# PARKCHEOLHEE-lab/building-gan-graph-conditioned-architectural-volume-generation

Measured on AMD Instinct MI355X. Metric: voxel-graphs/sec (full G+D step), higher is better.
Workload: dtype f32

## Files before the change

### building-gan-graph-conditioned-architectural-volume-generation_amd/csrc/gemm.hip

```cpp
#include "gemm_tile.h"

namespace {

using namespace vg::tile;

typedef float f32x16 __attribute__((ext_vector_type(16)));
typedef __bf16 bf16x4 __attribute__((ext_vector_type(4)));
typedef __bf16 bf16x8 __attribute__((ext_vector_type(8)));

constexpr int LDH = TK + 8;

__device__ __forceinline__ bf16x4 to_bf4(const float (&v)[4]) {
  bf16x4 r;
  r[0] = static_cast<__bf16>(v[0]);
  r[1] = static_cast<__bf16>(v[1]);
  r[2] = static_cast<__bf16>(v[2]);
  r[3] = static_cast<__bf16>(v[3]);
  return r;
}

__device__ __forceinline__ f32x16 mfma_bf(const __bf16* a, const __bf16* b, f32x16 acc) {
  return __builtin_amdgcn_mfma_f32_32x32x16_bf16(*reinterpret_cast<const bf16x8*>(a),
                                                 *reinterpret_cast<const bf16x8*>(b), acc, 0, 0, 0);
}
// ... 522 lines not shown
__global__ void __launch_bounds__(1024) k_gemm16(const float* __restrict__ A, int lda, const float* __restrict__ B,
                                                 int ldb, const float* __restrict__ bias,
                                                 const float* __restrict__ aux, int ldaux, float* __restrict__ C,
                                                 int ldc, int N, int M, int K,
                                                 const float* __restrict__ att_s = nullptr,
                                                 const float* __restrict__ att_d = nullptr,
                                                 float* __restrict__ a_src = nullptr,
                                                 float* __restrict__ a_dst = nullptr, const GnpDesc gn = GnpDesc{}) {
  gemm16_body<BT, ACT, ATT, BF, GNP, false, QA>(A, lda, B, ldb, bias, aux, ldaux, C, ldc, N, M, K, att_s, att_d,
                                                a_src, a_dst, gn);
}

template <bool BT, int ACT, bool ATT = false, bool BF = false, bool GNP = false, bool QA = false>
__global__ void __launch_bounds__(512) k_gemm8w(const float* __restrict__ A, int lda, const float* __restrict__ B,
                                                int ldb, const float* __restrict__ bias,
                                                const float* __restrict__ aux, int ldaux, float* __restrict__ C,
                                                int ldc, int N, int M, int K,
                                                const float* __restrict__ att_s = nullptr,
                                                const float* __restrict__ att_d = nullptr,
                                                float* __restrict__ a_src = nullptr,
                                                float* __restrict__ a_dst = nullptr, const GnpDesc gn = GnpDesc{}) {
  gemm16_body<BT, ACT, ATT, BF, GNP, false, QA, 8>(A, lda, B, ldb, bias, aux, ldaux, C, ldc, N, M, K, att_s, att_d,
                                                   a_src, a_dst, gn);
}

__global__ void __launch_bounds__(1024) __attribute__((amdgpu_waves_per_eu(8, 8)))
k_gemm16_gna(const float* __restrict__ A, const float* __restrict__ B, float* __restrict__ C, int N, int M, int K,
             const float* __restrict__ att_s, const float* __restrict__ att_d, float* __restrict__ a_src,
             float* __restrict__ a_dst, const GnaDesc ga) {
  gemm16_body<true, 0, true, false, false, true>(A, K, B, K, nullptr, nullptr, 0, C, M, N, M, K, att_s, att_d,
                                                 a_src, a_dst, GnpDesc{}, ga);
}

template <int NT, int TMR, bool ATT, int NTH>
__device__ __forceinline__ void ln_tile_epilogue(const float* Ct, float* s_mu, float* s_rs, int t, int n0, int N,
                                                 int M, const float* __restrict__ gamma,
                                                 const float* __restrict__ beta, float eps, float slope,
                                                 float* __restrict__ H, float* __restrict__ Y,
                                                 float* __restrict__ mean, float* __restrict__ rstd,
                                                 const float* __restrict__ att_s, const float* __restrict__ att_d,
                                                 float* __restrict__ a_src, float* __restrict__ a_dst, int ldy,
                                                 int s0 = 0) {
  constexpr int TNC = TN * NT;
  constexpr int CT = TNC + 1;
  if constexpr (ATT) {
    constexpr int TPR = NTH / TMR;
    constexpr int CPT = TNC / TPR;
    const int row = t / TPR, q = t % TPR;
    const float* cr = Ct + row * CT + q * CPT;
    float ss = 0.f, sd = 0.f;
#pragma unroll
    for (int i = 0; i < CPT; ++i) {
      const int c = q * CPT + i;
      if (c < M) {
        ss = fmaf(cr[i], att_s[c], ss);
        sd = fmaf(cr[i], att_d[c], sd);
      }
    }
#pragma unroll
    for (int off = 1; off < TPR; off <<= 1) {
      ss += __shfl_xor(ss, off, 64);
      sd += __shfl_xor(sd, off, 64);
    }
    if (q == 0 && n0 + row < N) {
      a_src[n0 + row] = ss;
      a_dst[n0 + row] = sd;
    }
    for (int idx = t; idx < TMR * TNC; idx += NTH) {
      const int r = idx / TNC, c = idx % TNC, n = n0 + r;
      if (c < M && n < N) H[(size_t)n * M + c] = Ct[r * CT + c];
    }
    return;
  }
  {
    constexpr int TPR = NTH / TMR;
    constexpr int CPT = TNC / TPR;
    const int row = t / TPR, q = t % TPR;
    const float* cr = Ct + row * CT + q * CPT;
    float v[CPT];
    float s = 0.f;
#pragma unroll
    for (int i = 0; i < CPT; ++i) {
      v[i] = q * CPT + i < M ? cr[i] : 0.f;
      s += v[i];
    }
#pragma unroll
    for (int off = 1; off < TPR; off <<= 1) s += __shfl_xor(s, off, 64);
    const float mu = s / static_cast<float>(M);
    float ss = 0.f;
#pragma unroll
    for (int i = 0; i < CPT; ++i)
      if (q * CPT + i < M) {
        const float d = v[i] - mu;
        ss = fmaf(d, d, ss);
      }
#pragma unroll
    for (int off = 1; off < TPR; off <<= 1) ss += __shfl_xor(ss, off, 64);
    const float rs = rsqrtf(ss / static_cast<float>(M) + eps);
    if (q == 0) {
      s_mu[row] = mu;
      s_rs[row] = rs;
      if (mean && n0 + row < N && n0 + row >= s0) {
        mean[n0 + row - s0] = mu;
        rstd[n0 + row - s0] = rs;
      }
    }
  }
  __syncthreads();
  for (int idx = t; idx < TMR * TNC; idx += NTH) {
    const int row = idx / TNC, c = idx % TNC, n = n0 + row;
    if (c < M && n < N) {
      const float v = Ct[row * CT + c];
      if (H && n >= s0) H[(size_t)(n - s0) * M + c] = v;
      const float z = fmaf((v - s_mu[row]) * s_rs[row], gamma[c], beta[c]);
      Y[(size_t)n * ldy + c] = z > 0.f ? z : z * slope;
    }
  }
}

constexpr int kMaxSrc = 4;
struct MsDesc {
  const float* p[kMaxSrc];
  int ld[kMaxSrc], kend[kMaxSrc], wcol[kMaxSrc], rmod[kMaxSrc];
  int nsrc;
  const float* add;
  int ld_add, add_rows;
  int s0 = 0;
};

template <int NT, int TMR = TM, bool ATT = false, bool MS = false, bool BF = false, bool QL = false>
__global__ void __launch_bounds__(256) k_gemm_ln(const float* __restrict__ A, int lda,
                                                 const float* __restrict__ B, int ldb,
                                                 const float* __restrict__ bias, int N, int M, int K,
                                                 const float* __restrict__ gamma,
                                                 const float* __restrict__ beta, float eps,
                                                 float slope, float* __restrict__ H,
                                                 float* __restrict__ Y, float* __restrict__ mean,
                                                 float* __restrict__ rstd,
                                                 const float* __restrict__ att_s = nullptr,
                                                 const float* __restrict__ att_d = nullptr,
                                                 float* __restrict__ a_src = nullptr,
                                                 float* __restrict__ a_dst = nullptr, int ldy = 0,
                                                 const MsDesc ms = MsDesc{}) {
  if (ldy == 0) ldy = M;
  constexpr int TNC = TN * NT;
  constexpr int CT = TNC + 1;
  constexpr int WCOLS = 4 / (TMR / 32);
  constexpr int NJ = TNC / (32 * WCOLS);
  static_assert(NJ >= 1, "TMR = 32 needs 128 columns");
  __shared__ __attribute__((aligned(16))) float smem[2 * TMR * LDP + 2 * TNC * LDP];
  __shared__ float s_mu[TMR], s_rs[TMR];
// ... 289 lines not shown
      const float* ar = As + buf * TMR * PIT + (wr * 16 + (lane & 15)) * LDP + (lane >> 4);
#pragma unroll
      for (int kk = 0; kk < TK; kk += 4)
#pragma unroll
        for (int j = 0; j < NJ; ++j)
          acc[j] = __builtin_amdgcn_mfma_f32_16x16x4f32(
              ar[kk], Bs[buf * TNC * PIT + (j * 16 * WCW + wc * 16 + (lane & 15)) * LDP + (lane >> 4) + kk], acc[j], 0,
              0, 0);
    }
    buf ^= 1;
  }
  __syncthreads();
  float* Ct = smem;
  const int add0 = MS && ms.add ? n0 % ms.add_rows : 0;
#pragma unroll
  for (int j = 0; j < NJ; ++j) {
    const int c = j * 16 * WCW + wc * 16 + (lane & 15);
    const float bv = (bias && c < M) ? bias[c] : 0.f;
#pragma unroll
    for (int r = 0; r < 4; ++r) {
      const int rl = wr * 16 + 4 * (lane >> 4) + r;
      float v = acc[j][r] + bv;
      if constexpr (MS) {
        if (ms.add && n0 + rl < N && c < M) {
          int ar2 = add0 + rl;
          if (ar2 >= ms.add_rows) ar2 -= ms.add_rows;
          v += ms.add[(size_t)ar2 * ms.ld_add + c];
        }
      }
      Ct[rl * CT + c] = v;
    }
  }
  __syncthreads();
  ln_tile_epilogue<NT, TMR, ATT, 1024>(Ct, s_mu, s_rs, t, n0, N, M, gamma, beta, eps, slope, H, Y, mean, rstd, att_s,
                                       att_d, a_src, a_dst, ldy, ms.s0);
}

template <int KT, bool MS>
__global__ void __launch_bounds__(1024) k_gemm_ln_wres(const float* __restrict__ A, int lda,
                                                       const float* __restrict__ B, int ldb,
                                                       const float* __restrict__ bias, int N, int M, int K,
                                                       const float* __restrict__ gamma,
                                                       const float* __restrict__ beta, float eps, float slope,
                                                       float* __restrict__ H, float* __restrict__ Y,
                                                       float* __restrict__ mean, float* __restrict__ rstd, int ldy,
                                                       const MsDesc ms) {
  constexpr int TMR = 32, NT = 2, TNC = TN * NT, CT = TNC + 1;
  constexpr int WRW = TMR / 16, WCW = 16 / WRW;
  static_assert(TNC / (16 * WCW) == 1, "one sub-tile per wave");
  constexpr int AIMG = TMR * FP, BIMG = TNC * FP;
  extern __shared__ float4 dyn4[];
  float* Ws = reinterpret_cast<float*>(dyn4);
  float* As = Ws + KT * BIMG;
  __shared__ float s_mu[TMR], s_rs[TMR];
  const int t = threadIdx.x, lane = t & 63, wave = t >> 6;
  const int wr = wave / WCW, wc = wave % WCW;
  const int kq4 = K / 4;
  const int tiles = (N + TMR - 1) / TMR;
  const int lb = xcd_remap(blockIdx.x, gridDim.x);
  const int t0 = (int)((long long)tiles * lb / gridDim.x), t1 = (int)((long long)tiles * (lb + 1) / gridDim.x);
  auto a_src = [&](int k, const float*& p, int& ld, int& col) {
    p = A;
    ld = lda;
    col = k;
    if constexpr (MS) {
      int sidx = 0;
#pragma unroll
      for (int i = 0; i < kMaxSrc - 1; ++i)
        if (i < ms.nsrc - 1 && k >= ms.kend[i]) sidx = i + 1;
      const int kb = sidx > 0 ? ms.kend[sidx - 1] : 0;
      p = ms.p[sidx];
      ld = ms.ld[sidx];
      col = k - kb;
    }
  };
  auto w_col = [&](int k) {
    if constexpr (MS) {
      int sidx = 0;
#pragma unroll
      for (int i = 0; i < kMaxSrc - 1; ++i)
        if (i < ms.nsrc - 1 && k >= ms.kend[i]) sidx = i + 1;
      const int kb = sidx > 0 ? ms.kend[sidx - 1] : 0;
      return ms.wcol[sidx] + (k - kb);
    }
    return k;
  };
  for (int g = t; g < TNC * kq4; g += 1024) {
    const int m = g / kq4, k = 4 * (g % kq4);
    const float4 v = m < M ? *reinterpret_cast<const float4*>(B + (size_t)m * ldb + w_col(k)) : make_float4(0.f, 0.f, 0.f, 0.f);
    float* d = Ws + (k >> 5) * BIMG;
    const int kk = k & 31;
    d[frag_pos(m, kk)] = v.x;
    d[frag_pos(m, kk + 1)] = v.y;
    d[frag_pos(m, kk + 2)] = v.z;
    d[frag_pos(m, kk + 3)] = v.w;
  }
  for (int g = t; g < TNC * (KT * 32 - K); g += 1024) {
    const int m = g / (KT * 32 - K), k = K + g % (KT * 32 - K);
    Ws[(k >> 5) * BIMG + frag_pos(m, k & 31)] = 0.f;
  }
  constexpr int QPT = (TMR * KT * 8 + 1023) / 1024;
  float4 qa[QPT];
  auto load_a = [&](int tile) {
    const int n0 = tile * TMR;
#pragma unroll
    for (int u = 0; u < QPT; ++u) {
      const int g = t + 1024 * u;
      const int r = g / kq4, k = 4 * (g % kq4);
      qa[u] = make_float4(0.f, 0.f, 0.f, 0.f);
      if (g < TMR * kq4 && n0 + r < N) {
        const float* p;
        int ld, col;
        a_src(k, p, ld, col);
        qa[u] = *reinterpret_cast<const float4*>(p + (size_t)(n0 + r) * ld + col);
      }
    }
  };
  auto store_a = [&]() {
#pragma unroll
    for (int u = 0; u < QPT; ++u) {
      const int g = t + 1024 * u;
      if (g < TMR * kq4) {
        const int r = g / kq4, k = 4 * (g % kq4);
        float* d = As + (k >> 5) * AIMG;
        const int kk = k & 31;
        d[frag_pos(r, kk)] = qa[u].x;
        d[frag_pos(r, kk + 1)] = qa[u].y;
        d[frag_pos(r, kk + 2)] = qa[u].z;
        d[frag_pos(r, kk + 3)] = qa[u].w;
      }
    }
    for (int g = t; g < TMR * (KT * 32 - K); g += 1024) {
      const int r = g / (KT * 32 - K), k = K + g % (KT * 32 - K);
      As[(k >> 5) * AIMG + frag_pos(r, k & 31)] = 0.f;
    }
  };
  if (t0 < t1) {
    load_a(t0);
    store_a();
  }
  const int c = wc * 16 + (lane & 15);
  const float bv = (bias && c < M) ? bias[c] : 0.f;
  __syncthreads();
  for (int tile = t0; tile < t1; ++tile) {
    const int n0 = tile * TMR;
    if (tile + 1 < t1) load_a(tile + 1);
    f32x4 acc = f32x4{0.f, 0.f, 0.f, 0.f};
    const int ra_ = wr * 16 + (lane & 15), g = lane >> 4;
#pragma unroll
    for (int kt = 0; kt < KT; ++kt) {
      const float* Ai = As + kt * AIMG;
      const float* Bi = Ws + kt * BIMG;
      const float4 a0 = *reinterpret_cast<const float4*>(Ai + frag_at(ra_, g, 0));
      const float4 a1 = *reinterpret_cast<const float4*>(Ai + frag_at(ra_, g, 1));
      const float av[8] = {a0.x, a0.y, a0.z, a0.w, a1.x, a1.y, a1.z, a1.w};
      const float4 b0 = *reinterpret_cast<const float4*>(Bi + frag_at(c, g, 0));
      const float4 b1 = *reinterpret_cast<const float4*>(Bi + frag_at(c, g, 1));
      const float bw[8] = {b0.x, b0.y, b0.z, b0.w, b1.x, b1.y, b1.z, b1.w};
#pragma unroll
      for (int i = 0; i < 8; ++i) acc = __builtin_amdgcn_mfma_f32_16x16x4f32(av[i], bw[i], acc, 0, 0, 0);
    }
    __syncthreads();
    float* Ct = As;
    const int add0 = MS && ms.add ? n0 % ms.add_rows : 0;
#pragma unroll
    for (int r = 0; r < 4; ++r) {
      const int rl = wr * 16 + 4 * (lane >> 4) + r;
      float v = acc[r] + bv;
      if constexpr (MS) {
        if (ms.add && n0 + rl < N && c < M) {
          int ar2 = add0 + rl;
          if (ar2 >= ms.add_rows) ar2 -= ms.add_rows;
          v += ms.add[(size_t)ar2 * ms.ld_add + c];
        }
      }
      Ct[rl * CT + c] = v;
    }
    __syncthreads();
    ln_tile_epilogue<NT, TMR, false, 1024>(Ct, s_mu, s_rs, t, n0, N, M, gamma, beta, eps, slope, H, Y, mean, rstd,
                                           nullptr, nullptr, nullptr, nullptr, ldy, ms.s0);
    __syncthreads();
    if (tile + 1 < t1) store_a();
    __syncthreads();
  }
}

template <int KT>
constexpr int wres_lds_bytes() {
  return (KT * TN * 2 * FP + (KT * 32 * FP > 32 * (2 * TN + 1) ? KT * 32 * FP : 32 * (2 * TN + 1))) * 4;
}

template <int G>
constexpr int tn_smem_floats() { return G * 2 * TK * (TM + 1) + G * 2 * TK * (TN + 1); }

template <int G, bool BF>
__device__ __forceinline__ void tn_tile(float* smem, const float* __restrict__ A, int lda, const float* __restrict__ B,
                                        int ldb, int N, int M, int K, int rows, int chunk, int m0, int k0,
                                        float* __restrict__ part, float* __restrict__ pdb, int db_rows) {
  float(*As)[2][TK][TM + 1] = reinterpret_cast<float(*)[2][TK][TM + 1]>(smem);
  float(*Bs)[2][TK][TN + 1] = reinterpret_cast<float(*)[2][TK][TN + 1]>(smem + G * 2 * TK * (TM + 1));
  constexpr int PER = (TK * TM) / 256;
  const int grp = threadIdx.x >> 8, t = threadIdx.x & 255, lane = t & 63, wave = t >> 6;
  const int wr = wave >> 1, wc = wave & 1;
  const int nb = chunk * rows, ne = min(N, nb + rows);
  const int steps = ne > nb ? (ne - nb + TK - 1) / TK : 0;
  const int iters = (steps + G - 1) / G;
  const bool do_db = pdb && k0 == 0;
  f32x16 acc;
#pragma unroll
  for (int r = 0; r < 16; ++r) acc[r] = 0.f;
  float dbs = 0.f;
  __bf16(*Ah)[2][TM][LDH] = reinterpret_cast<__bf16(*)[2][TM][LDH]>(smem);
  __bf16(*Bh)[2][TN][LDH] = reinterpret_cast<__bf16(*)[2][TN][LDH]>(smem + G * 2 * TK * (TM + 1));
  float ra[PER], rb[PER];
  auto load = [&](int st) {
    const int n1 = nb + st * TK;
#pragma unroll
    for (int q = 0; q < PER; ++q) {
      const int e = t + 256 * q;
      const int c = e % TM;
      const int r = BF ? 4 * ((t >> 6) + 4 * (q >> 2)) + (q & 3) : e / TM;
      const int n = n1 + r;
// ... 789 lines not shown
    k_gemm_tn_group<kTnGroups, true><<<static_cast<int>(blocks), 256 * kTnGroups, 0, s>>>(g);
  else
    k_gemm_tn_group<kTnGroups, false><<<static_cast<int>(blocks), 256 * kTnGroups, 0, s>>>(g);
  VG_CHECK_LAUNCH();
  return 0;
}

static inline bool al16(const void* p) { return (reinterpret_cast<uintptr_t>(p) & 15) == 0; }

#ifndef VG_WRES
#define VG_WRES 1
#endif
#ifndef VG_LN_TM64_K
#define VG_LN_TM64_K 384
#endif
#ifndef VG_WRES_MIN_ROWS
#define VG_WRES_MIN_ROWS 16384
#endif
static int wres_cus() {
  static int cus = 0;
  if (!cus) {
    int dev = 0, n = 0;
    if (hipGetDevice(&dev) != hipSuccess || hipDeviceGetAttribute(&n, hipDeviceAttributeMultiprocessorCount, dev) !=
                                                  hipSuccess || n <= 0)
      n = 256;
    cus = n;
  }
  return cus;
}

template <int KT, bool MS>
static void launch_wres(const float* A, int lda, const float* W, int ldw, const float* bias, int N, int M, int K,
                        const float* gamma, const float* beta, float eps, float slope, float* H, float* Y, float* mean,
                        float* rstd, int ldy, const MsDesc& d, hipStream_t s) {
  static bool attr = false;
  constexpr int bytes = wres_lds_bytes<KT>();
  if (!attr) {
    (void)hipFuncSetAttribute(reinterpret_cast<const void*>(&k_gemm_ln_wres<KT, MS>),
                              hipFuncAttributeMaxDynamicSharedMemorySize, bytes);
    attr = true;
  }
  const int tiles = (N + 31) / 32;
  const int grid = tiles < wres_cus() ? tiles : wres_cus();
  k_gemm_ln_wres<KT, MS><<<grid, 1024, bytes, s>>>(A, lda, W, ldw, bias, N, M, K, gamma, beta, eps, slope, H, Y, mean,
                                                   rstd, ldy, d);
}

template <bool MS>
static bool try_wres(const float* A, int lda, const float* W, int ldw, const float* bias, int N, int M, int K,
                     const float* gamma, const float* beta, float eps, float slope, float* H, float* Y, float* mean,
                     float* rstd, int ldy, const MsDesc& d, hipStream_t s) {
  if (!VG_WRES || N < VG_WRES_MIN_ROWS || M <= TN || M > 2 * TN || K % 4 || K <= 0) return false;
  switch ((K + 31) / 32) {
    case 1: launch_wres<1, MS>(A, lda, W, ldw, bias, N, M, K, gamma, beta, eps, slope, H, Y, mean, rstd, ldy, d, s); return true;
    case 2: launch_wres<2, MS>(A, lda, W, ldw, bias, N, M, K, gamma, beta, eps, slope, H, Y, mean, rstd, ldy, d, s); return true;
    case 3: launch_wres<3, MS>(A, lda, W, ldw, bias, N, M, K, gamma, beta, eps, slope, H, Y, mean, rstd, ldy, d, s); return true;
    case 4: launch_wres<4, MS>(A, lda, W, ldw, bias, N, M, K, gamma, beta, eps, slope, H, Y, mean, rstd, ldy, d, s); return true;
    case 5: launch_wres<5, MS>(A, lda, W, ldw, bias, N, M, K, gamma, beta, eps, slope, H, Y, mean, rstd, ldy, d, s); return true;
    default: return false;
  }
}

template <bool BF>
static int gemm_ln_act(const float* A, int32_t lda, const float* W, int32_t N, int32_t M,
                       int32_t K, const float* bias, const float* gamma, const float* beta,
                       float eps, float slope, float* H, float* Y, float* mean, float* rstd,
                       void* stream, int32_t s0 = 0) {
  if (N < 0 || M <= 0 || M > 2 * TN || K <= 0 || lda < K || !A || !W || !gamma || !beta || !Y ||
      ((mean == nullptr) != (rstd == nullptr)) || s0 < 0 || (s0 > 0 && s0 >= N))
    return VG_EINVAL;
  MsDesc d{};
  d.s0 = s0;
  if (N == 0) return 0;
  hipStream_t s = static_cast<hipStream_t>(stream);
  const dim3 grid((N + TM - 1) / TM, 1);
  const bool ql = VG_QUAD_A && K % 4 == 0 && lda % 4 == 0 && al16(A) && al16(W);
  if (!BF && ql && try_wres<false>(A, lda, W, K, bias, N, M, K, gamma, beta, eps, slope, H, Y, mean, rstd, M, d, s)) {
  } else if (!BF && VG_LN16) {
    if (M <= TN && ql)
      k_gemm_ln16<1, TM, false, false, true><<<grid, 1024, 0, s>>>(A, lda, W, K, bias, N, M, K, gamma, beta, eps,
                                                                  slope, H, Y, mean, rstd,
                                                                  nullptr, nullptr, nullptr, nullptr, 0, d);
    else if (M <= TN)
      k_gemm_ln16<1, TM><<<grid, 1024, 0, s>>>(A, lda, W, K, bias, N, M, K, gamma, beta, eps, slope, H, Y, mean,
                                              rstd, nullptr, nullptr, nullptr, nullptr, 0, d);
    else if (VG_LN_TM32 && ql && K >= VG_LN_TM64_K)
      k_gemm_ln16<2, TM, false, false, true><<<grid, 1024, 0, s>>>(A, lda, W, K, bias, N, M, K, gamma, beta, eps,
                                                                  slope, H, Y, mean, rstd,
                                                                  nullptr, nullptr, nullptr, nullptr, 0, d);
    else if (VG_LN_TM32 && ql)
      k_gemm_ln16<2, 32, false, false, true><<<dim3((N + 31) / 32, 1), 1024, 0, s>>>(
          A, lda, W, K, bias, N, M, K, gamma, beta, eps, slope, H, Y, mean, rstd,
          nullptr, nullptr, nullptr, nullptr, 0, d);
// ... 89 lines not shown
        nullptr, nullptr, ldy, d);
  else if (!BF && VG_LN16)
    k_gemm_ln16<2, 32, false, true><<<dim3((N + 31) / 32, 1), 1024, 0, s>>>(
        nullptr, 0, W, ldw, bias, N, M, K, gamma, beta, eps, slope, nullptr, Y, nullptr, nullptr, nullptr, nullptr,
        nullptr, nullptr, ldy, d);
  else if (BF && ql)
    k_gemm_ln<2, 32, false, true, BF, BF><<<dim3((N + 31) / 32, 1), 256, 0, s>>>(
        nullptr, 0, W, ldw, bias, N, M, K, gamma, beta, eps, slope, nullptr, Y, nullptr, nullptr, nullptr, nullptr,
        nullptr, nullptr, ldy, d);
  else
    k_gemm_ln<2, 32, false, true, BF><<<dim3((N + 31) / 32, 1), 256, 0, s>>>(
        nullptr, 0, W, ldw, bias, N, M, K, gamma, beta, eps, slope, nullptr, Y, nullptr, nullptr, nullptr, nullptr,
        nullptr, nullptr, ldy, d);
  VG_CHECK_LAUNCH();
  return 0;
}

extern "C" int vg_gemm_ln_act_ms(const vg_asrc* src, int32_t nsrc, const float* W, int32_t ldw, int32_t N,
                                 int32_t M, const float* bias, const float* addend, int32_t ld_add,
                                 int32_t add_rows, const float* gamma, const float* beta, float eps, float slope,
                                 float* Y, int32_t ldy, void* stream) {
  return gemm_ln_act_ms<false>(src, nsrc, W, ldw, N, M, bias, addend, ld_add, add_rows, gamma, beta, eps, slope,
                               Y, ldy, stream);
}

extern "C" int vg_gemm_ln_act_ms_bf16(const vg_asrc* src, int32_t nsrc, const float* W, int32_t ldw, int32_t N,
                                      int32_t M, const float* bias, const float* addend, int32_t ld_add,
                                      int32_t add_rows, const float* gamma, const float* beta, float eps,
                                      float slope, float* Y, int32_t ldy, void* stream) {
  return gemm_ln_act_ms<true>(src, nsrc, W, ldw, N, M, bias, addend, ld_add, add_rows, gamma, beta, eps, slope,
                              Y, ldy, stream);
}

template <bool BF>
static int gat_lin_att(const float* X, int32_t ldx, const float* W, int32_t N,
                       int32_t Cin, int32_t C, const float* att_src, const float* att_dst,
                       float* H, float* a_src, float* a_dst, void* stream) {
  if (N < 0 || Cin <= 0 || C <= 0 || ldx < Cin || !X || !W || !att_src || !att_dst || !H ||
      !a_src || !a_dst)
    return VG_EINVAL;
  if (N == 0) return 0;
  hipStream_t s = static_cast<hipStream_t>(stream);
  if (C > 2 * TN) {
    const int rc = gemm<BF>(X, ldx, W, Cin, 1, nullptr, 0, nullptr, 0, H, C, N, C, Cin, stream);
    if (rc) return rc;
    return vg_gat_att(H, N, C, att_src, att_dst, a_src, a_dst, stream);
  }
  if (C > TN) {
    if (!BF && VG_LN16 && quad_ab(X, ldx, W, Cin, Cin, C, true))
      k_gemm_ln16<2, 32, true, false, true><<<dim3((N + 31) / 32, 1), 1024, 0, s>>>(
          X, ldx, W, Cin, nullptr, N, C, Cin, nullptr, nullptr, 0.f, 0.f, H, nullptr, nullptr, nullptr, att_src,
          att_dst, a_src, a_dst);
    else if (!BF && VG_LN16)
      k_gemm_ln16<2, 32, true><<<dim3((N + 31) / 32, 1), 1024, 0, s>>>(
          X, ldx, W, Cin, nullptr, N, C, Cin, nullptr, nullptr, 0.f, 0.f, H, nullptr, nullptr, nullptr, att_src,
          att_dst, a_src, a_dst);
    else
      k_gemm_ln<2, 32, true, false, BF><<<dim3((N + 31) / 32, 1), 256, 0, s>>>(
          X, ldx, W, Cin, nullptr, N, C, Cin, nullptr, nullptr, 0.f, 0.f, H, nullptr, nullptr, nullptr, att_src,
          att_dst, a_src, a_dst);
    VG_CHECK_LAUNCH();
    return 0;
  }
  if ((VG_GEMM16 & 2) && (!BF || (VG_GEMM16 & 8)))
    if (quad_ab(X, ldx, W, Cin, Cin, C, true))
      if (use_8w(dim3((N + TM - 1) / TM, 1)))
// ... 93 lines not shown
```

### building-gan-graph-conditioned-architectural-volume-generation_amd/vgan/_lib.py

```python
from __future__ import annotations

import ctypes
import os
from typing import Optional

import torch

LIB_PATH = os.environ.get("VGAN_LIB") or os.path.join(os.path.dirname(os.path.abspath(__file__)), "libvgan_hip.so")
VG_EINVAL = -1
VG_SELECT_MAX_COPIES = 64
VG_SELECT_F1, VG_SELECT_FAR = 0, 1

_c_i32, _c_i64, _c_f32, _c_p = ctypes.c_int32, ctypes.c_int64, ctypes.c_float, ctypes.c_void_p



class VgFoldSrc(ctypes.Structure):
    _fields_ = [("part", _c_p), ("rows", _c_i32), ("ld", _c_i32)]


class VgFold(ctypes.Structure):
    _fields_ = [("out", _c_p), ("width", _c_i32), ("k", _c_i32), ("ldo", _c_i32), ("accumulate", _c_i32),
                ("nsrc", _c_i32), ("src", VgFoldSrc * 2)]

# ... 247 lines not shown
                                       _c_p, _c_p, _c_p]),
    "vg_hgat_gna_max_segments": (_c_i32, []),
    "vg_hgat_lin_att_gn": (ctypes.c_int, [_c_p, _c_i32, _c_p, _c_i32, _c_i32, _c_i32, _c_i32, _c_p, _c_p, _c_p,
                                          _c_i32, _c_p, _c_p, _c_p, _c_p, _c_p, _c_p, _c_i32, _c_i32, _c_i32, _c_p]),
    "vg_hgat_fwd": (ctypes.c_int, [_c_p, _c_p, _c_i32, _c_i32, _c_i32, _c_p, _c_p, _c_p, _c_p, _c_f32, _c_p, _c_i32,
                                   _c_p]),
    "vg_graphnorm_fwd_h": (ctypes.c_int, [_c_p, _c_i32, _c_i32, _c_i32, _c_i32, _c_p, _c_p, _c_p, _c_f32, _c_p,
                                          _c_i32, _c_p, _c_p, _c_p]),
    "vg_hgat_gnp_rows": (_c_i32, [_c_i32, _c_i32]),
    "vg_hgat_gnp_floats": (_c_i64, [_c_i32, _c_i32]),
    "vg_hgat_fwd_gnp": (ctypes.c_int, [_c_p, _c_p, _c_i32, _c_i32, _c_i32, _c_p, _c_p, _c_p, _c_p, _c_f32, _c_p,
                                       _c_i32, _c_i32, _c_p, _c_p]),
    "vg_graphnorm_fwd_h_gnp": (ctypes.c_int, [_c_p, _c_i32, _c_i32, _c_i32, _c_i32, _c_p, _c_p, _c_p, _c_f32, _c_p,
                                              _c_i32, _c_p, _c_p, _c_i32, _c_p]),
    "vg_rng_fill": (ctypes.c_int, [_c_p, _c_i64, _c_i32, ctypes.c_uint64, _c_p, ctypes.c_uint32, _c_p]),
    "vg_rng_fill_at": (ctypes.c_int, [_c_p, _c_i64, _c_i32, ctypes.c_uint64, _c_p, _c_i64, ctypes.c_uint32, _c_p]),
    "vg_graphnorm_fwd_drop_tail": (ctypes.c_int, [_c_p, _c_i32, _c_i32, _c_i32, _c_p, _c_p, _c_p, _c_f32,
                                                  ctypes.c_uint64, _c_p, ctypes.c_uint32, _c_f32, _c_p, _c_p, _c_p, _c_p,
                                                  ctypes.POINTER(VgDrawTail), _c_p]),
    "vg_graphnorm_fwd_gnp_tail": (ctypes.c_int, [_c_p, _c_i32, _c_i32, _c_i32, _c_p, _c_p, _c_p, _c_f32,
                                                 ctypes.c_uint64, _c_p, ctypes.c_uint32, _c_f32, _c_p, _c_p, _c_p, _c_p,
                                                 _c_i32, ctypes.POINTER(VgDrawTail), _c_p]),
    "vg_gemm_ln_act_from": (ctypes.c_int, [_c_p, _c_i32, _c_p, _c_i32, _c_i32, _c_i32, _c_p, _c_p, _c_p, _c_f32,
                                           _c_f32, _c_i32, _c_p, _c_p, _c_p, _c_p, _c_p]),
    "vg_gen_state_bytes": (ctypes.c_int64, []),
    "vg_gen_hoist_arena_floats": (ctypes.c_int64, [ctypes.POINTER(VgGenModel), ctypes.POINTER(VgGenBatch),
                                                   ctypes.POINTER(VgGenStack)]),
    "vg_gen_forward_stacked": (ctypes.c_int, [ctypes.POINTER(VgGenModel), ctypes.POINTER(VgGenBatch),
                                              ctypes.POINTER(VgGenStack), _c_p, _c_i64, _c_p, _c_p, _c_p, _c_p]),
    "vg_gen_loss_and_grad_from": (ctypes.c_int, [ctypes.POINTER(VgGenModel), ctypes.POINTER(VgGenBatch), _c_p, _c_p,
                                                 _c_i64, _c_p, _c_p]),
    "vg_gemm_ln_act_ms": (ctypes.c_int, [_c_p, _c_i32, _c_p, _c_i32, _c_i32, _c_i32, _c_p, _c_p, _c_i32, _c_i32, _c_p,
                                         _c_p, _c_f32, _c_f32, _c_p, _c_i32, _c_p]),
    "vg_csr_ws_ints": (_c_i64, [_c_i64, _c_i32]),
    "vg_csr_build": (ctypes.c_int, [_c_p, _c_i64, _c_i32, _c_p, _c_p, _c_p, _c_p, _c_p, _c_p, _c_p, _c_p]),
    "vg_gat_fwd": (ctypes.c_int, [_c_p, _c_p, _c_i32, _c_i32, _c_p, _c_p, _c_p, _c_p, _c_f32, _c_p, _c_p, _c_p,
                                  _c_p, _c_p]),
    "vg_gat_att": (ctypes.c_int, [_c_p, _c_i32, _c_i32, _c_p, _c_p, _c_p, _c_p, _c_p]),
    "vg_gat_lin_att": (ctypes.c_int, [_c_p, _c_i32, _c_p, _c_i32, _c_i32, _c_i32, _c_p, _c_p, _c_p, _c_p, _c_p,
                                      _c_p]),
    "vg_csr_ell": (ctypes.c_int, [_c_p, _c_p, _c_i32, _c_i32, _c_p, _c_p]),
    "vg_gat_aggregate_fwd_ell": (ctypes.c_int, [_c_p, _c_p, _c_p, _c_i32, _c_i32, _c_i32, _c_p, _c_p, _c_p, _c_p,
                                                _c_f32, _c_p, _c_p, _c_p]),
    "vg_gat_lin_att_gn": (ctypes.c_int, [_c_p, _c_p, _c_i32, _c_i32, _c_i32, _c_p, _c_p, _c_p, _c_p, _c_p,
                                         ctypes.POINTER(VgGnApply), _c_p]),
    "vg_graphnorm_stats_gnp": (ctypes.c_int, [_c_i32, _c_i32, _c_i32, _c_p, _c_i32, _c_p, _c_f32, _c_p, _c_p]),
    "vg_graphnorm_stats": (ctypes.c_int, [_c_p, _c_i32, _c_i32, _c_i32, _c_p, _c_f32, _c_p, _c_p, _c_p]),
    "vg_gat_jvp2_blocks": (_c_i32, [_c_i32, _c_i32]),
    "vg_gat_jvp2_gn_deferred": (ctypes.c_int, [_c_p] * 5 + [_c_i32] * 3 + [_c_p] * 8 + [_c_f32] + [_c_p] * 7 +
                                [ctypes.POINTER(VgGnJvp), _c_p, _c_p, _c_p]),
    "vg_graphnorm_jvp2_part": (ctypes.c_int, [_c_p, _c_i32, _c_i32, _c_p, _c_p, _c_p, _c_p, _c_f32, _c_p, _c_p, _c_p,
                                              _c_p, _c_p, _c_p, _c_p, _c_p, _c_i32, _c_p, _c_p]),
    "vg_linear_chain": (ctypes.c_int, [_c_p, _c_i32, _c_i32, _c_p, _c_i32, _c_p, _c_p]),
    "vg_graph_exec_update": (ctypes.c_int, [_c_p, _c_p]),
    "vg_graph_launch": (ctypes.c_int, [_c_p, _c_p]),
    "vg_hgen_arena_bytes": (ctypes.c_int64, [ctypes.POINTER(VgHgenModel), ctypes.POINTER(VgHgenBatch)]),
    "vg_hgen_sweep": (ctypes.c_int, [ctypes.POINTER(VgHgenModel), ctypes.POINTER(VgHgenBatch), _c_p, ctypes.c_int64,
                                     _c_p, _c_p, _c_p]),
    "vg_hgen_graph_create": (_c_p, []),
    "vg_hgen_graph_destroy": (None, [_c_p]),
    "vg_hgen_graph_stats": (ctypes.c_int, [_c_p, ctypes.POINTER(_c_i32), ctypes.POINTER(_c_i32)]),
    "vg_hgen_sweep_graphed": (ctypes.c_int, [_c_p, ctypes.POINTER(VgHgenModel), ctypes.POINTER(VgHgenBatch), _c_p,
                                             ctypes.c_int64, _c_p, _c_p, _c_p]),
    "vg_critic_arena_floats": (ctypes.c_int64, [ctypes.POINTER(VgCriticModel), ctypes.POINTER(VgCriticBatch)]),
    "vg_critic_loss_and_grad": (ctypes.c_int, [ctypes.POINTER(VgCriticModel), ctypes.POINTER(VgCriticBatch), _c_p,
                                               _c_i64, _c_p, _c_p]),
# ... 332 lines not shown
```

### include/vgan.h

```cpp
#ifndef VGAN_H_
#define VGAN_H_

#include <stdint.h>
#include <stddef.h>

#ifdef __cplusplus
extern "C" {
#endif

#define VG_EINVAL (-1)
#define VG_EGRAPH_TOPOLOGY (-2)


int64_t vg_csr_ws_ints(int64_t num_edges, int32_t num_nodes);

int vg_csr_build(const int64_t* edge_index, int64_t num_edges, int32_t num_nodes,
                 int32_t* row_ptr, int32_t* col, int32_t* csc_ptr, int32_t* csc_slot,
                 int32_t* csc_dst, int32_t* workspace, int32_t* status, void* stream);


int vg_gat_fwd(const int32_t* row_ptr, const int32_t* col, int32_t num_nodes, int32_t channels,
               const float* h, const float* att_src, const float* att_dst, const float* bias,
               float slope, float* out, float* alpha, float* a_src, float* a_dst, void* stream);

// ... 386 lines not shown
                            const float* g_y, float* u_out, float* x_inj, const float* workspace, void* stream);


typedef struct vg_chain_layer {
  const float* weight;
  const float* bias;
  const float* aux;
  float* out;
  int32_t ld_aux;
  int32_t ld_out;
  int32_t w_trans;
  int32_t act;
} vg_chain_layer;

int vg_linear_chain(const float* x, int32_t ldx, int32_t rows, const int32_t* widths, int32_t nlayers,
                    const vg_chain_layer* layers, void* stream);
int vg_linear_chain_bf16(const float* x, int32_t ldx, int32_t rows, const int32_t* widths, int32_t nlayers,
                         const vg_chain_layer* layers, void* stream);


typedef struct vg_asrc {
  const float* ptr;
  int32_t ld;
  int32_t cols;
  int32_t w_col0;
  int32_t rows_mod;
} vg_asrc;

int vg_gemm_ln_act_ms(const vg_asrc* src, int32_t nsrc, const float* W, int32_t ldw, int32_t N,
                      int32_t M, const float* bias, const float* addend, int32_t ld_add,
                      int32_t add_rows, const float* gamma, const float* beta, float eps, float slope,
                      float* Y, int32_t ldy, void* stream);


int vg_csr_ell(const int32_t* row_ptr, const int32_t* col, int32_t num_nodes, int32_t width, int32_t* ell,
               void* stream);
int vg_gat_aggregate_fwd_ell(const int32_t* row_ptr, const int32_t* col, const int32_t* ell, int32_t ell_width,
                             int32_t num_nodes, int32_t channels, const float* h, const float* a_src,
                             const float* a_dst, const float* bias, float slope, float* out, float* alpha,
                             void* stream);
int32_t vg_gat_gnp_rows(int32_t num_nodes, int32_t channels);
int32_t vg_gat_fwd_sliced(int32_t num_nodes, int32_t channels);
int64_t vg_gat_gnp_floats(int32_t num_nodes, int32_t channels);
int vg_gat_aggregate_fwd_gnp(const int32_t* row_ptr, const int32_t* col, const int32_t* ell, int32_t ell_width,
                             int32_t num_nodes, int32_t channels, const float* h, const float* a_src,
                             const float* a_dst, const float* bias, float slope, float* out, float* alpha,
                             int32_t seg_rows, float* gnp, void* stream);

int64_t vg_gat_tile_plan_ints(int32_t num_nodes, int32_t num_edges);
int vg_gat_tile_plan(const int32_t* row_ptr, const int32_t* col, int32_t num_nodes,
                     int32_t num_edges, int32_t* plan_out, void* stream);

int vg_gat_aggregate_fwd_lds(const int32_t* row_ptr, const int32_t* col, int32_t num_nodes,
                             int32_t channels, const float* h, const float* a_src,
                             const float* a_dst, const float* bias, float slope, float* out,
                             float* alpha, const int32_t* plan, int32_t umax, void* stream);

const char* vg_build_stamp(void);

int64_t vg_gat_stage_plan_ints(int32_t num_nodes, int32_t num_edges);
int vg_gat_stage_plan(const int32_t* row_ptr, const int32_t* col, int32_t num_nodes, int32_t num_edges,
                      int32_t* plan_out, void* stream);

int vg_gat_aggregate_fwd_staged(const int32_t* row_ptr, const int32_t* col, int32_t num_nodes, int32_t channels,
                                const float* h, const float* a_src, const float* a_dst, const float* bias,
                                float slope, float* out, float* alpha, const int32_t* plan, void* stream);
// ... 393 lines not shown
```

Baseline: 4592.

## Double-buffer weight-resident GEMM+LayerNorm kernel and move LN epilogue into registers

```diff
diff --git a/building-gan-graph-conditioned-architectural-volume-generation_amd/csrc/gemm.hip b/building-gan-graph-conditioned-architectural-volume-generation_amd/csrc/gemm.hip
--- a/building-gan-graph-conditioned-architectural-volume-generation_amd/csrc/gemm.hip
+++ b/building-gan-graph-conditioned-architectural-volume-generation_amd/csrc/gemm.hip
@@ -578,6 +578,21 @@
                                                  a_src, a_dst, GnpDesc{}, ga);
 }
 
+#ifndef VG_WRES_STAMPS
+#define VG_WRES_STAMPS 0
+#endif
+#if VG_WRES_STAMPS
+__device__ unsigned long long* g_wres_stamps = nullptr;
+__device__ int g_wres_stamp_cap = 0;
+__device__ __forceinline__ void wres_stamp(int& k, int tag) {
+  if (threadIdx.x == 0 && blockIdx.x == 0 && g_wres_stamps && k < g_wres_stamp_cap)
+    g_wres_stamps[k] = (wall_clock64() << 8) | static_cast<unsigned long long>(tag);
+  ++k;
+}
+#else
+__device__ __forceinline__ void wres_stamp(int&, int) {}
+#endif
+
 template <int NT, int TMR, bool ATT, int NTH>
 __device__ __forceinline__ void ln_tile_epilogue(const float* Ct, float* s_mu, float* s_rs, int t, int n0, int N,
                                                  int M, const float* __restrict__ gamma,
@@ -586,7 +601,7 @@
                                                  float* __restrict__ mean, float* __restrict__ rstd,
                                                  const float* __restrict__ att_s, const float* __restrict__ att_d,
                                                  float* __restrict__ a_src, float* __restrict__ a_dst, int ldy,
-                                                 int s0 = 0) {
+                                                 int s0 = 0, int* stamp_k = nullptr) {
   constexpr int TNC = TN * NT;
   constexpr int CT = TNC + 1;
   if constexpr (ATT) {
@@ -653,6 +668,7 @@
     }
   }
   __syncthreads();
+  if (VG_WRES_STAMPS && stamp_k) wres_stamp(*stamp_k, 3);
   for (int idx = t; idx < TMR * TNC; idx += NTH) {
     const int row = idx / TNC, c = idx % TNC, n = n0 + row;
     if (c < M && n < N) {
@@ -663,6 +679,88 @@
     }
   }
 }
+
+#ifndef VG_LN_EPI_REG
+#define VG_LN_EPI_REG 1
+#endif
+#ifndef VG_LN16_EPI_REG
+#define VG_LN16_EPI_REG 0
+#endif
+template <int NT, int TMR, int NTH>
+struct LnReg {
+  static constexpr int TNC = TN * NT, CT = TNC + 1, TPR = NTH / TMR, CPT = TNC / TPR;
+  static_assert(CPT % 4 == 0 && CPT <= 8, "whole quads per lane");
+  float gm[CPT], bt[CPT];
+  bool vy, vh;
+  __device__ __forceinline__ void init(int t, int M, const float* __restrict__ gamma, const float* __restrict__ beta,
+                                       const float* H, const float* Y, int ldy) {
+    const int c0 = (t % TPR) * CPT;
+#pragma unroll
+    for (int i = 0; i < CPT; ++i) {
+      gm[i] = c0 + i < M ? gamma[c0 + i] : 0.f;
+      bt[i] = c0 + i < M ? beta[c0 + i] : 0.f;
+    }
+    vy = (reinterpret_cast<uintptr_t>(Y) & 15) == 0 && ldy % 4 == 0;
+    vh = (reinterpret_cast<uintptr_t>(H) & 15) == 0 && M % 4 == 0;
+  }
+  __device__ __forceinline__ void run(const float* Ct, int t, int n0, int N, int M, float eps, float slope,
+                                      float* __restrict__ H, float* __restrict__ Y, float* __restrict__ mean,
+                                      float* __restrict__ rstd, int ldy, int s0) const {
+    const int row = t / TPR, q = t % TPR, c0 = q * CPT, n = n0 + row;
+    const float* cr = Ct + row * CT + c0;
+    float v[CPT];
+    float s = 0.f;
+#pragma unroll
+    for (int i = 0; i < CPT; ++i) {
+      v[i] = c0 + i < M ? cr[i] : 0.f;
+      s += v[i];
+    }
+#pragma unroll
+    for (int off = 1; off < TPR; off <<= 1) s += __shfl_xor(s, off, 64);
+    const float mu = s / static_cast<float>(M);
+    float ss = 0.f;
+#pragma unroll
+    for (int i = 0; i < CPT; ++i)
+      if (c0 + i < M) {
+        const float d = v[i] - mu;
+        ss = fmaf(d, d, ss);
+      }
+#pragma unroll
+    for (int off = 1; off < TPR; off <<= 1) ss += __shfl_xor(ss, off, 64);
+    const float rs = rsqrtf(ss / static_cast<float>(M) + eps);
+    if (n >= N) return;
+    if (q == 0 && mean && n >= s0) {
+      mean[n - s0] = mu;
+      rstd[n - s0] = rs;
+    }
+    float* yr = Y + (size_t)n * ldy + c0;
+    float* hr = (H && n >= s0) ? H + (size_t)(n - s0) * M + c0 : nullptr;
+#pragma unroll
+    for (int j = 0; j < CPT; j += 4) {
+      float z[4];
+#pragma unroll
+      for (int i = 0; i < 4; ++i) {
+        const float u = fmaf((v[j + i] - mu) * rs, gm[j + i], bt[j + i]);
+        z[i] = u > 0.f ? u : u * slope;
+      }
+      const bool full = c0 + j + 3 < M;
+      if (hr) {
+        if (full && vh)
+          *reinterpret_cast<f32x4*>(hr + j) = f32x4{v[j], v[j + 1], v[j + 2], v[j + 3]};
+        else
+#pragma unroll
+          for (int i = 0; i < 4; ++i)
+            if (c0 + j + i < M) hr[j + i] = v[j + i];
+      }
+      if (full && vy)
+        *reinterpret_cast<f32x4*>(yr + j) = f32x4{z[0], z[1], z[2], z[3]};
+      else
+#pragma unroll
+        for (int i = 0; i < 4; ++i)
+          if (c0 + j + i < M) yr[j + i] = z[i];
+    }
+  }
+};
 
 constexpr int kMaxSrc = 4;
 struct MsDesc {
@@ -1018,9 +1116,28 @@
     }
   }
   __syncthreads();
-  ln_tile_epilogue<NT, TMR, ATT, 1024>(Ct, s_mu, s_rs, t, n0, N, M, gamma, beta, eps, slope, H, Y, mean, rstd, att_s,
-                                       att_d, a_src, a_dst, ldy, ms.s0);
-}
+  if constexpr (VG_LN16_EPI_REG && !ATT) {
+    LnReg<NT, TMR, 1024> ep;
+    ep.init(t, M, gamma, beta, H, Y, ldy);
+    ep.run(Ct, t, n0, N, M, eps, slope, H, Y, mean, rstd, ldy, ms.s0);
+  } else {
+    ln_tile_epilogue<NT, TMR, ATT, 1024>(Ct, s_mu, s_rs, t, n0, N, M, gamma, beta, eps, slope, H, Y, mean, rstd,
+                                         att_s, att_d, a_src, a_dst, ldy, ms.s0);
+  }
+}
+
+#ifndef VG_WRES_PIPE
+#define VG_WRES_PIPE 1
+#endif
+#ifndef VG_WRES_PRO
+#define VG_WRES_PRO 1
+#endif
+template <int KT>
+constexpr int wres_region_floats() {
+  return KT * 32 * FP > 32 * (2 * TN + 1) ? KT * 32 * FP : 32 * (2 * TN + 1);
+}
+template <int KT>
+constexpr bool wres_pipe() { return VG_WRES_PIPE != 0 && VG_LN_EPI_REG != 0 && KT <= 4; }
 
 template <int KT, bool MS>
 __global__ void __launch_bounds__(1024) k_gemm_ln_wres(const float* __restrict__ A, int lda,
@@ -1037,8 +1154,10 @@
   constexpr int AIMG = TMR * FP, BIMG = TNC * FP;
   extern __shared__ float4 dyn4[];
   float* Ws = reinterpret_cast<float*>(dyn4);
-  float* As = Ws + KT * BIMG;
-  __shared__ float s_mu[TMR], s_rs[TMR];
+  float* R0 = Ws + KT * BIMG;
+  constexpr int AREG = wres_region_floats<KT>();
+  constexpr bool REG = VG_LN_EPI_REG, PIPE = wres_pipe<KT>();
+  __shared__ float s_mu[REG ? 1 : TMR], s_rs[REG ? 1 : TMR];
   const int t = threadIdx.x, lane = t & 63, wave = t >> 6;
   const int wr = wave / WCW, wc = wave % WCW;
   const int kq4 = K / 4;
@@ -1071,20 +1190,33 @@
     }
     return k;
   };
-  for (int g = t; g < TNC * kq4; g += 1024) {
-    const int m = g / kq4, k = 4 * (g % kq4);
-    const float4 v = m < M ? *reinterpret_cast<const float4*>(B + (size_t)m * ldb + w_col(k)) : make_float4(0.f, 0.f, 0.f, 0.f);
-    float* d = Ws + (k >> 5) * BIMG;
-    const int kk = k & 31;
-    d[frag_pos(m, kk)] = v.x;
-    d[frag_pos(m, kk + 1)] = v.y;
-    d[frag_pos(m, kk + 2)] = v.z;
-    d[frag_pos(m, kk + 3)] = v.w;
-  }
-  for (int g = t; g < TNC * (KT * 32 - K); g += 1024) {
-    const int m = g / (KT * 32 - K), k = K + g % (KT * 32 - K);
-    Ws[(k >> 5) * BIMG + frag_pos(m, k & 31)] = 0.f;
-  }
+  auto stage_w = [&]() {
+    float4 wq[KT];
+#pragma unroll
+    for (int u = 0; u < KT; ++u) {
+      const int g = t + 1024 * u;
+      const int m = g / kq4, k = 4 * (g % kq4);
+      wq[u] = (g < TNC * kq4 && m < M) ? *reinterpret_cast<const float4*>(B + (size_t)m * ldb + w_col(k))
+                                       : make_float4(0.f, 0.f, 0.f, 0.f);
+    }
+#pragma unroll
+    for (int u = 0; u < KT; ++u) {
+      const int g = t + 1024 * u;
+      if (g < TNC * kq4) {
+        const int m = g / kq4, k = 4 * (g % kq4);
+        float* d = Ws + (k >> 5) * BIMG;
+        const int kk = k & 31;
+        d[frag_pos(m, kk)] = wq[u].x;
+        d[frag_pos(m, kk + 1)] = wq[u].y;
+        d[frag_pos(m, kk + 2)] = wq[u].z;
+        d[frag_pos(m, kk + 3)] = wq[u].w;
+      }
+    }
+    for (int g = t; g < TNC * (KT * 32 - K); g += 1024) {
+      const int m = g / (KT * 32 - K), k = K + g % (KT * 32 - K);
+      Ws[(k >> 5) * BIMG + frag_pos(m, k & 31)] = 0.f;
+    }
+  };
   constexpr int QPT = (TMR * KT * 8 + 1023) / 1024;
   float4 qa[QPT];
   auto load_a = [&](int tile) {
@@ -1102,7 +1234,7 @@
       }
     }
   };
-  auto store_a = [&]() {
+  auto store_a = [&](float* As) {
 #pragma unroll
     for (int u = 0; u < QPT; ++u) {
       const int g = t + 1024 * u;
@@ -1121,16 +1253,9 @@
       As[(k >> 5) * AIMG + frag_pos(r, k & 31)] = 0.f;
     }
   };
-  if (t0 < t1) {
-    load_a(t0);
-    store_a();
-  }
   const int c = wc * 16 + (lane & 15);
   const float bv = (bias && c < M) ? bias[c] : 0.f;
-  __syncthreads();
-  for (int tile = t0; tile < t1; ++tile) {
-    const int n0 = tile * TMR;
-    if (tile + 1 < t1) load_a(tile + 1);
+  auto mfma_tile = [&](const float* As) {
     f32x4 acc = f32x4{0.f, 0.f, 0.f, 0.f};
     const int ra_ = wr * 16 + (lane & 15), g = lane >> 4;
 #pragma unroll
@@ -1146,8 +1271,9 @@
 #pragma unroll
       for (int i = 0; i < 8; ++i) acc = __builtin_amdgcn_mfma_f32_16x16x4f32(av[i], bw[i], acc, 0, 0, 0);
     }
-    __syncthreads();
-    float* Ct = As;
+    return acc;
+  };
+  auto stage = [&](float* Ct, const f32x4& acc, int n0) {
     const int add0 = MS && ms.add ? n0 % ms.add_rows : 0;
 #pragma unroll
     for (int r = 0; r < 4; ++r) {
@@ -1162,18 +1288,84 @@
       }
       Ct[rl * CT + c] = v;
     }
-    __syncthreads();
-    ln_tile_epilogue<NT, TMR, false, 1024>(Ct, s_mu, s_rs, t, n0, N, M, gamma, beta, eps, slope, H, Y, mean, rstd,
-                                           nullptr, nullptr, nullptr, nullptr, ldy, ms.s0);
-    __syncthreads();
-    if (tile + 1 < t1) store_a();
-    __syncthreads();
+  };
+  [[maybe_unused]] int sk = 0;
+  if constexpr (PIPE) {
+    const int T = t1 - t0;
+    LnReg<NT, TMR, 1024> ep;
+    ep.init(t, M, gamma, beta, H, Y, ldy);
+    if (VG_WRES_PRO != 0 && T > 0) load_a(t0);
+    stage_w();
+    if (T > 0) {
+      if (VG_WRES_PRO == 0) load_a(t0);
+      store_a(R0);
+      if (T > 1) load_a(t0 + 1);
+    }
+    __syncthreads();
+    if (T <= 0) return;
+    wres_stamp(sk, 0);
+    f32x4 acc = mfma_tile(R0);
+    __syncthreads();
+    wres_stamp(sk, 5);
+    stage(R0, acc, t0 * TMR);
+    if (T > 1) store_a(R0 + AREG);
+    if (T > 2) load_a(t0 + 2);
+    __syncthreads();
+    wres_stamp(sk, 6);
+    for (int i = 0; i + 1 < T; ++i) {
+      float* Ri = R0 + (i & 1) * AREG;
+      float* Rn = R0 + ((i + 1) & 1) * AREG;
+      acc = mfma_tile(Rn);
+      ep.run(Ri, t, (t0 + i) * TMR, N, M, eps, slope, H, Y, mean, rstd, ldy, ms.s0);
+      __syncthreads();
+      wres_stamp(sk, 5);
+      stage(Rn, acc, (t0 + i + 1) * TMR);
+      if (i + 2 < T) store_a(Ri);
+      if (i + 3 < T) load_a(t0 + i + 3);
+      __syncthreads();
+      wres_stamp(sk, 6);
+    }
+    ep.run(R0 + ((T - 1) & 1) * AREG, t, (t0 + T - 1) * TMR, N, M, eps, slope, H, Y, mean, rstd, ldy, ms.s0);
+    wres_stamp(sk, 7);
+  } else {
+    float* As = R0;
+    [[maybe_unused]] LnReg<NT, TMR, 1024> ep;
+    if constexpr (REG) ep.init(t, M, gamma, beta, H, Y, ldy);
+    stage_w();
+    if (t0 < t1) {
+      load_a(t0);
+      store_a(As);
+    }
+    __syncthreads();
+    wres_stamp(sk, 0);
+    for (int tile = t0; tile < t1; ++tile) {
+      const int n0 = tile * TMR;
+      if (tile + 1 < t1) load_a(tile + 1);
+      const f32x4 acc = mfma_tile(As);
+      __syncthreads();
+      wres_stamp(sk, 1);
+      float* Ct = As;
+      stage(Ct, acc, n0);
+      __syncthreads();
+      wres_stamp(sk, 2);
+      if constexpr (REG)
+        ep.run(Ct, t, n0, N, M, eps, slope, H, Y, mean, rstd, ldy, ms.s0);
+      else
+        ln_tile_epilogue<NT, TMR, false, 1024>(Ct, s_mu, s_rs, t, n0, N, M, gamma, beta, eps, slope, H, Y, mean, rstd,
+                                               nullptr, nullptr, nullptr, nullptr, ldy, ms.s0,
+                                               VG_WRES_STAMPS ? &sk : nullptr);
+      __syncthreads();
+      wres_stamp(sk, 4);
+      if (tile + 1 < t1) store_a(As);
+      __syncthreads();
+      wres_stamp(sk, 8);
+    }
   }
 }
 
 template <int KT>
 constexpr int wres_lds_bytes() {
-  return (KT * TN * 2 * FP + (KT * 32 * FP > 32 * (2 * TN + 1) ? KT * 32 * FP : 32 * (2 * TN + 1))) * 4;
+  return (KT * TN * 2 * FP + (wres_pipe<KT>() ? 2 : 1) * wres_region_floats<KT>()) * 4;
 }
 
 template <int G>
@@ -2029,7 +2221,7 @@
 template <int KT, bool MS>
 static void launch_wres(const float* A, int lda, const float* W, int ldw, const float* bias, int N, int M, int K,
                         const float* gamma, const float* beta, float eps, float slope, float* H, float* Y, float* mean,
-                        float* rstd, int ldy, const MsDesc& d, hipStream_t s) {
+                        float* rstd, int ldy, const MsDesc& d, hipStream_t s, int workgroups = 0) {
   static bool attr = false;
   constexpr int bytes = wres_lds_bytes<KT>();
   if (!attr) {
@@ -2038,24 +2230,33 @@
     attr = true;
   }
   const int tiles = (N + 31) / 32;
-  const int grid = tiles < wres_cus() ? tiles : wres_cus();
+  const int want = workgroups > 0 ? workgroups : wres_cus();
+  const int grid = tiles < want ? tiles : want;
   k_gemm_ln_wres<KT, MS><<<grid, 1024, bytes, s>>>(A, lda, W, ldw, bias, N, M, K, gamma, beta, eps, slope, H, Y, mean,
                                                    rstd, ldy, d);
+}
+
+template <bool MS>
+static bool run_wres(const float* A, int lda, const float* W, int ldw, const float* bias, int N, int M, int K,
+                     const float* gamma, const float* beta, float eps, float slope, float* H, float* Y, float* mean,
+                     float* rstd, int ldy, const MsDesc& d, hipStream_t s, int workgroups = 0) {
+  if (N <= 0 || M <= TN || M > 2 * TN || K % 4 || K <= 0) return false;
+  switch ((K + 31) / 32) {
+    case 1: launch_wres<1, MS>(A, lda, W, ldw, bias, N, M, K, gamma, beta, eps, slope, H, Y, mean, rstd, ldy, d, s, workgroups); return true;
+    case 2: launch_wres<2, MS>(A, lda, W, ldw, bias, N, M, K, gamma, beta, eps, slope, H, Y, mean, rstd, ldy, d, s, workgroups); return true;
+    case 3: launch_wres<3, MS>(A, lda, W, ldw, bias, N, M, K, gamma, beta, eps, slope, H, Y, mean, rstd, ldy, d, s, workgroups); return true;
+    case 4: launch_wres<4, MS>(A, lda, W, ldw, bias, N, M, K, gamma, beta, eps, slope, H, Y, mean, rstd, ldy, d, s, workgroups); return true;
+    case 5: launch_wres<5, MS>(A, lda, W, ldw, bias, N, M, K, gamma, beta, eps, slope, H, Y, mean, rstd, ldy, d, s, workgroups); return true;
+    default: return false;
+  }
 }
 
 template <bool MS>
 static bool try_wres(const float* A, int lda, const float* W, int ldw, const float* bias, int N, int M, int K,
                      const float* gamma, const float* beta, float eps, float slope, float* H, float* Y, float* mean,
                      float* rstd, int ldy, const MsDesc& d, hipStream_t s) {
-  if (!VG_WRES || N < VG_WRES_MIN_ROWS || M <= TN || M > 2 * TN || K % 4 || K <= 0) return false;
-  switch ((K + 31) / 32) {
-    case 1: launch_wres<1, MS>(A, lda, W, ldw, bias, N, M, K, gamma, beta, eps, slope, H, Y, mean, rstd, ldy, d, s); return true;
-    case 2: launch_wres<2, MS>(A, lda, W, ldw, bias, N, M, K, gamma, beta, eps, slope, H, Y, mean, rstd, ldy, d, s); return true;
-    case 3: launch_wres<3, MS>(A, lda, W, ldw, bias, N, M, K, gamma, beta, eps, slope, H, Y, mean, rstd, ldy, d, s); return true;
-    case 4: launch_wres<4, MS>(A, lda, W, ldw, bias, N, M, K, gamma, beta, eps, slope, H, Y, mean, rstd, ldy, d, s); return true;
-    case 5: launch_wres<5, MS>(A, lda, W, ldw, bias, N, M, K, gamma, beta, eps, slope, H, Y, mean, rstd, ldy, d, s); return true;
-    default: return false;
-  }
+  if (!VG_WRES || N < VG_WRES_MIN_ROWS) return false;
+  return run_wres<MS>(A, lda, W, ldw, bias, N, M, K, gamma, beta, eps, slope, H, Y, mean, rstd, ldy, d, s);
 }
 
 template <bool BF>
@@ -2211,6 +2412,59 @@
                               Y, ldy, stream);
 }
 
+extern "C" int vg_gemm_ln_act_wres(const vg_asrc* src, int32_t nsrc, const float* W, int32_t ldw, int32_t N,
+                                   int32_t M, const float* bias, const float* addend, int32_t ld_add,
+                                   int32_t add_rows, const float* gamma, const float* beta, float eps, float slope,
+                                   int32_t first_row, float* H, float* Y, int32_t ldy, float* mean, float* rstd,
+                                   int32_t workgroups, void* stream) {
+  if (!src || nsrc <= 0 || nsrc > kMaxSrc || !W || N < 0 || M <= TN || M > 2 * TN || !gamma || !beta || !Y ||
+      ldy < M || (addend && (ld_add < M || add_rows < 32)) || ((mean == nullptr) != (rstd == nullptr)) ||
+      first_row < 0 || (first_row > 0 && first_row >= N) || workgroups <= 0 || ldw % 4 || !al16(W))
+    return VG_EINVAL;
+  const bool ms = nsrc > 1 || addend;
+  MsDesc d{};
+  int K = 0;
+  for (int i = 0; i < nsrc; ++i) {
+    if (!src[i].ptr || src[i].cols <= 0 || src[i].cols % (ms ? TK : 4) || src[i].ld < src[i].cols ||
+        src[i].w_col0 < 0 || src[i].w_col0 + src[i].cols > ldw || src[i].rows_mod != 0 || src[i].ld % 4 ||
+        src[i].w_col0 % 4 || !al16(src[i].ptr))
+      return VG_EINVAL;
+    K += src[i].cols;
+    d.p[i] = src[i].ptr;
+    d.ld[i] = src[i].ld;
+    d.kend[i] = K;
+    d.wcol[i] = src[i].w_col0;
+    d.rmod[i] = src[i].rows_mod;
+  }
+  if (K > 160) return VG_EINVAL;
+  d.nsrc = nsrc;
+  d.add = addend;
+  d.ld_add = ld_add;
+  d.add_rows = add_rows;
+  d.s0 = first_row;
+  if (N == 0) return 0;
+  hipStream_t s = static_cast<hipStream_t>(stream);
+  const bool ok = ms ? run_wres<true>(nullptr, 0, W, ldw, bias, N, M, K, gamma, beta, eps, slope, H, Y, mean, rstd,
+                                      ldy, d, s, workgroups)
+                     : run_wres<false>(src[0].ptr, src[0].ld, W + src[0].w_col0, ldw, bias, N, M, K, gamma, beta,
+                                       eps, slope, H, Y, mean, rstd, ldy, d, s, workgroups);
+  if (!ok) return VG_EINVAL;
+  VG_CHECK_LAUNCH();
+  return 0;
+}
+#if VG_WRES_STAMPS
+extern "C" int vg_wres_stamps(unsigned long long* buf, int32_t cap, int32_t* khz) {
+  int dev = 0, rate = 0;
+  if (hipGetDevice(&dev) != hipSuccess ||
+      hipDeviceGetAttribute(&rate, hipDeviceAttributeWallClockRate, dev) != hipSuccess ||
+      hipMemcpyToSymbol(HIP_SYMBOL(g_wres_stamps), &buf, sizeof(buf)) != hipSuccess ||
+      hipMemcpyToSymbol(HIP_SYMBOL(g_wres_stamp_cap), &cap, sizeof(cap)) != hipSuccess)
+    return VG_EINVAL;
+  if (khz) *khz = rate;
+  return 0;
+}
+#endif
+
 template <bool BF>
 static int gat_lin_att(const float* X, int32_t ldx, const float* W, int32_t N,
                        int32_t Cin, int32_t C, const float* att_src, const float* att_dst,
diff --git a/building-gan-graph-conditioned-architectural-volume-generation_amd/vgan/_lib.py b/building-gan-graph-conditioned-architectural-volume-generation_amd/vgan/_lib.py
--- a/building-gan-graph-conditioned-architectural-volume-generation_amd/vgan/_lib.py
+++ b/building-gan-graph-conditioned-architectural-volume-generation_amd/vgan/_lib.py
@@ -303,6 +303,9 @@
                                                  _c_i64, _c_p, _c_p]),
     "vg_gemm_ln_act_ms": (ctypes.c_int, [_c_p, _c_i32, _c_p, _c_i32, _c_i32, _c_i32, _c_p, _c_p, _c_i32, _c_i32, _c_p,
                                          _c_p, _c_f32, _c_f32, _c_p, _c_i32, _c_p]),
+    "vg_gemm_ln_act_wres": (ctypes.c_int, [_c_p, _c_i32, _c_p, _c_i32, _c_i32, _c_i32, _c_p, _c_p, _c_i32, _c_i32,
+                                           _c_p, _c_p, _c_f32, _c_f32, _c_i32, _c_p, _c_p, _c_i32, _c_p, _c_p, _c_i32,
+                                           _c_p]),
     "vg_csr_ws_ints": (_c_i64, [_c_i64, _c_i32]),
     "vg_csr_build": (ctypes.c_int, [_c_p, _c_i64, _c_i32, _c_p, _c_p, _c_p, _c_p, _c_p, _c_p, _c_p, _c_p]),
     "vg_gat_fwd": (ctypes.c_int, [_c_p, _c_p, _c_i32, _c_i32, _c_p, _c_p, _c_p, _c_p, _c_f32, _c_p, _c_p, _c_p,
diff --git a/include/vgan.h b/include/vgan.h
--- a/include/vgan.h
+++ b/include/vgan.h
@@ -442,6 +442,12 @@
                       int32_t add_rows, const float* gamma, const float* beta, float eps, float slope,
                       float* Y, int32_t ldy, void* stream);
 
+int vg_gemm_ln_act_wres(const vg_asrc* src, int32_t nsrc, const float* W, int32_t ldw, int32_t N,
+                        int32_t M, const float* bias, const float* addend, int32_t ld_add,
+                        int32_t add_rows, const float* gamma, const float* beta, float eps, float slope,
+                        int32_t first_row, float* H, float* Y, int32_t ldy, float* mean, float* rstd,
+                        int32_t workgroups, void* stream);
+
 
 int vg_csr_ell(const int32_t* row_ptr, const int32_t* col, int32_t num_nodes, int32_t width, int32_t* ell,
                void* stream);
```

New measurement: 4631 (median of 6 runs). Within noise of the previous version (+0.8%).
